# microsoft/MaskFlownet

Hardware: NVIDIA H100
Metric: image-pairs/sec (MaskFlownet-S forward, 1024x448) (higher is better)
Workload: dtype f32

## Files before the change

maskflownet_b200/csrc/conv3x3_wgmma.cu:

```cuda
#include <cstring>
#include <type_traits>

#include "mma_tiles.cuh"
#include "split_act.cuh"

namespace mfn {
namespace um {
constexpr int MT_WIDE = 128, MT_NARROW = 64;
inline int tile_width(int OW, int stride) {
  return tuning().conv_narrow && (OW <= MT_NARROW || (stride == 2 && tuning().conv_tma_in)) ? MT_NARROW : MT_WIDE;
}
constexpr int R = 2;
constexpr int NTHREADS = 384;
constexpr int NCONS = 8;
constexpr int NPROD = 3;
constexpr int MAX_AS = 4, MAX_WS = 24;
constexpr int MAX_RS = 4;
constexpr int BATCH = 6;
constexpr int BAR_BYTES = 1024;

__host__ __device__ inline int n_slots(int stride, int dil) { return stride == 2 ? 2 * R + 1 : (dil >= R ? 3 * R : R + 2 * dil); }
__host__ __device__ inline int row_pitch(int mt, int stride, int dil) { return stride == 2 ? 2 * mt + 1 : mt + 2 * dil; }
__host__ __device__ inline int slot_of(int r, int ky, int stride, int dil) {
  return stride == 2 ? 2 * r + ky : (dil >= R ? ky * R + r : r + ky * dil);
// ... 51 lines not shown
      : "+f"(d[0]), "+f"(d[1]), "+f"(d[2]), "+f"(d[3]), "+f"(d[4]), "+f"(d[5]), "+f"(d[6]), "+f"(d[7]), "+f"(d[8]), "+f"(d[9]), "+f"(d[10]), "+f"(d[11]), "+f"(d[12]), "+f"(d[13]), "+f"(d[14]), "+f"(d[15]), "+f"(d[16]), "+f"(d[17]), "+f"(d[18]), "+f"(d[19]), "+f"(d[20]), "+f"(d[21]), "+f"(d[22]), "+f"(d[23])
      : "l"(a), "l"(b), "r"(scale_d));
}
template <int S>
__device__ __forceinline__ void wgmma_n64(float (&d)[S], uint64_t a, uint64_t b, uint32_t scale_d) {
  static_assert(S >= 32, "accumulator too small");
  asm volatile(
      "{\n\t.reg .pred p;\n\tsetp.ne.b32 p, %34, 0;\n\t"
      "wgmma.mma_async.sync.aligned.m64n64k16.f32.bf16.bf16 {%0, %1, %2, %3, %4, %5, %6, %7, %8, %9, %10, %11, %12, %13, %14, %15, %16, %17, %18, %19, %20, %21, %22, %23, %24, %25, %26, %27, %28, %29, %30, %31}, %32, %33, p, 1, 1, 0, 0;\n\t}"
      : "+f"(d[0]), "+f"(d[1]), "+f"(d[2]), "+f"(d[3]), "+f"(d[4]), "+f"(d[5]), "+f"(d[6]), "+f"(d[7]), "+f"(d[8]), "+f"(d[9]), "+f"(d[10]), "+f"(d[11]), "+f"(d[12]), "+f"(d[13]), "+f"(d[14]), "+f"(d[15]), "+f"(d[16]), "+f"(d[17]), "+f"(d[18]), "+f"(d[19]), "+f"(d[20]), "+f"(d[21]), "+f"(d[22]), "+f"(d[23]), "+f"(d[24]), "+f"(d[25]), "+f"(d[26]), "+f"(d[27]), "+f"(d[28]), "+f"(d[29]), "+f"(d[30]), "+f"(d[31])
      : "l"(a), "l"(b), "r"(scale_d));
}
template <int S>
__device__ __forceinline__ void wgmma_n80(float (&d)[S], uint64_t a, uint64_t b, uint32_t scale_d) {
  static_assert(S >= 40, "accumulator too small");
  asm volatile(
      "{\n\t.reg .pred p;\n\tsetp.ne.b32 p, %42, 0;\n\t"
      "wgmma.mma_async.sync.aligned.m64n80k16.f32.bf16.bf16 {%0, %1, %2, %3, %4, %5, %6, %7, %8, %9, %10, %11, %12, %13, %14, %15, %16, %17, %18, %19, %20, %21, %22, %23, %24, %25, %26, %27, %28, %29, %30, %31, %32, %33, %34, %35, %36, %37, %38, %39}, %40, %41, p, 1, 1, 0, 0;\n\t}"
      : "+f"(d[0]), "+f"(d[1]), "+f"(d[2]), "+f"(d[3]), "+f"(d[4]), "+f"(d[5]), "+f"(d[6]), "+f"(d[7]), "+f"(d[8]), "+f"(d[9]), "+f"(d[10]), "+f"(d[11]), "+f"(d[12]), "+f"(d[13]), "+f"(d[14]), "+f"(d[15]), "+f"(d[16]), "+f"(d[17]), "+f"(d[18]), "+f"(d[19]), "+f"(d[20]), "+f"(d[21]), "+f"(d[22]), "+f"(d[23]), "+f"(d[24]), "+f"(d[25]), "+f"(d[26]), "+f"(d[27]), "+f"(d[28]), "+f"(d[29]), "+f"(d[30]), "+f"(d[31]), "+f"(d[32]), "+f"(d[33]), "+f"(d[34]), "+f"(d[35]), "+f"(d[36]), "+f"(d[37]), "+f"(d[38]), "+f"(d[39])
      : "l"(a), "l"(b), "r"(scale_d));
}
template <int S>
__device__ __forceinline__ void wgmma_n96(float (&d)[S], uint64_t a, uint64_t b, uint32_t scale_d) {
  static_assert(S >= 48, "accumulator too small");
  asm volatile(
      "{\n\t.reg .pred p;\n\tsetp.ne.b32 p, %50, 0;\n\t"
      "wgmma.mma_async.sync.aligned.m64n96k16.f32.bf16.bf16 {%0, %1, %2, %3, %4, %5, %6, %7, %8, %9, %10, %11, %12, %13, %14, %15, %16, %17, %18, %19, %20, %21, %22, %23, %24, %25, %26, %27, %28, %29, %30, %31, %32, %33, %34, %35, %36, %37, %38, %39, %40, %41, %42, %43, %44, %45, %46, %47}, %48, %49, p, 1, 1, 0, 0;\n\t}"
      : "+f"(d[0]), "+f"(d[1]), "+f"(d[2]), "+f"(d[3]), "+f"(d[4]), "+f"(d[5]), "+f"(d[6]), "+f"(d[7]), "+f"(d[8]), "+f"(d[9]), "+f"(d[10]), "+f"(d[11]), "+f"(d[12]), "+f"(d[13]), "+f"(d[14]), "+f"(d[15]), "+f"(d[16]), "+f"(d[17]), "+f"(d[18]), "+f"(d[19]), "+f"(d[20]), "+f"(d[21]), "+f"(d[22]), "+f"(d[23]), "+f"(d[24]), "+f"(d[25]), "+f"(d[26]), "+f"(d[27]), "+f"(d[28]), "+f"(d[29]), "+f"(d[30]), "+f"(d[31]), "+f"(d[32]), "+f"(d[33]), "+f"(d[34]), "+f"(d[35]), "+f"(d[36]), "+f"(d[37]), "+f"(d[38]), "+f"(d[39]), "+f"(d[40]), "+f"(d[41]), "+f"(d[42]), "+f"(d[43]), "+f"(d[44]), "+f"(d[45]), "+f"(d[46]), "+f"(d[47])
      : "l"(a), "l"(b), "r"(scale_d));
}
template <int S>
__device__ __forceinline__ void wgmma_n112(float (&d)[S], uint64_t a, uint64_t b, uint32_t scale_d) {
  static_assert(S >= 56, "accumulator too small");
  asm volatile(
      "{\n\t.reg .pred p;\n\tsetp.ne.b32 p, %58, 0;\n\t"
      "wgmma.mma_async.sync.aligned.m64n112k16.f32.bf16.bf16 {%0, %1, %2, %3, %4, %5, %6, %7, %8, %9, %10, %11, %12, %13, %14, %15, %16, %17, %18, %19, %20, %21, %22, %23, %24, %25, %26, %27, %28, %29, %30, %31, %32, %33, %34, %35, %36, %37, %38, %39, %40, %41, %42, %43, %44, %45, %46, %47, %48, %49, %50, %51, %52, %53, %54, %55}, %56, %57, p, 1, 1, 0, 0;\n\t}"
      : "+f"(d[0]), "+f"(d[1]), "+f"(d[2]), "+f"(d[3]), "+f"(d[4]), "+f"(d[5]), "+f"(d[6]), "+f"(d[7]), "+f"(d[8]), "+f"(d[9]), "+f"(d[10]), "+f"(d[11]), "+f"(d[12]), "+f"(d[13]), "+f"(d[14]), "+f"(d[15]), "+f"(d[16]), "+f"(d[17]), "+f"(d[18]), "+f"(d[19]), "+f"(d[20]), "+f"(d[21]), "+f"(d[22]), "+f"(d[23]), "+f"(d[24]), "+f"(d[25]), "+f"(d[26]), "+f"(d[27]), "+f"(d[28]), "+f"(d[29]), "+f"(d[30]), "+f"(d[31]), "+f"(d[32]), "+f"(d[33]), "+f"(d[34]), "+f"(d[35]), "+f"(d[36]), "+f"(d[37]), "+f"(d[38]), "+f"(d[39]), "+f"(d[40]), "+f"(d[41]), "+f"(d[42]), "+f"(d[43]), "+f"(d[44]), "+f"(d[45]), "+f"(d[46]), "+f"(d[47]), "+f"(d[48]), "+f"(d[49]), "+f"(d[50]), "+f"(d[51]), "+f"(d[52]), "+f"(d[53]), "+f"(d[54]), "+f"(d[55])
      : "l"(a), "l"(b), "r"(scale_d));
}
template <int S>
__device__ __forceinline__ void wgmma_n128(float (&d)[S], uint64_t a, uint64_t b, uint32_t scale_d) {
  static_assert(S >= 64, "accumulator too small");
  asm volatile(
      "{\n\t.reg .pred p;\n\tsetp.ne.b32 p, %66, 0;\n\t"
      "wgmma.mma_async.sync.aligned.m64n128k16.f32.bf16.bf16 {%0, %1, %2, %3, %4, %5, %6, %7, %8, %9, %10, %11, %12, %13, %14, %15, %16, %17, %18, %19, %20, %21, %22, %23, %24, %25, %26, %27, %28, %29, %30, %31, %32, %33, %34, %35, %36, %37, %38, %39, %40, %41, %42, %43, %44, %45, %46, %47, %48, %49, %50, %51, %52, %53, %54, %55, %56, %57, %58, %59, %60, %61, %62, %63}, %64, %65, p, 1, 1, 0, 0;\n\t}"
      : "+f"(d[0]), "+f"(d[1]), "+f"(d[2]), "+f"(d[3]), "+f"(d[4]), "+f"(d[5]), "+f"(d[6]), "+f"(d[7]), "+f"(d[8]), "+f"(d[9]), "+f"(d[10]), "+f"(d[11]), "+f"(d[12]), "+f"(d[13]), "+f"(d[14]), "+f"(d[15]), "+f"(d[16]), "+f"(d[17]), "+f"(d[18]), "+f"(d[19]), "+f"(d[20]), "+f"(d[21]), "+f"(d[22]), "+f"(d[23]), "+f"(d[24]), "+f"(d[25]), "+f"(d[26]), "+f"(d[27]), "+f"(d[28]), "+f"(d[29]), "+f"(d[30]), "+f"(d[31]), "+f"(d[32]), "+f"(d[33]), "+f"(d[34]), "+f"(d[35]), "+f"(d[36]), "+f"(d[37]), "+f"(d[38]), "+f"(d[39]), "+f"(d[40]), "+f"(d[41]), "+f"(d[42]), "+f"(d[43]), "+f"(d[44]), "+f"(d[45]), "+f"(d[46]), "+f"(d[47]), "+f"(d[48]), "+f"(d[49]), "+f"(d[50]), "+f"(d[51]), "+f"(d[52]), "+f"(d[53]), "+f"(d[54]), "+f"(d[55]), "+f"(d[56]), "+f"(d[57]), "+f"(d[58]), "+f"(d[59]), "+f"(d[60]), "+f"(d[61]), "+f"(d[62]), "+f"(d[63])
      : "l"(a), "l"(b), "r"(scale_d));
}
template <int N, int S>
__device__ __forceinline__ void wgmma_bf16(float (&d)[S], uint64_t a, uint64_t b, uint32_t scale_d) {
  if constexpr (N == 16) wgmma_n16(d, a, b, scale_d);
  else if constexpr (N == 32) wgmma_n32(d, a, b, scale_d);
  else if constexpr (N == 48) wgmma_n48(d, a, b, scale_d);
  else if constexpr (N == 64) wgmma_n64(d, a, b, scale_d);
  else if constexpr (N == 80) wgmma_n80(d, a, b, scale_d);
  else if constexpr (N == 96) wgmma_n96(d, a, b, scale_d);
  else if constexpr (N == 112) wgmma_n112(d, a, b, scale_d);
  else wgmma_n128(d, a, b, scale_d);
}

struct SplitK {
  int k, from, n_lo, y_lo, rh;
  long long part_stride;
  float* ws;
  uint32_t magic_tp, magic_tx;
  int as_wide;
  int ns;
  int stg;
};
__device__ __forceinline__ void decode_tile(int tile, int tilesX, int tilesY, const SplitK& sk, int& tx, int& ty, int& n) {
  if (sk.magic_tp) {
    n = (int)__umulhi((uint32_t)tile, sk.magic_tp);
    const int rem = tile - n * tilesX * tilesY;
    ty = sk.magic_tx ? (int)__umulhi((uint32_t)rem, sk.magic_tx) : rem;
    tx = rem - ty * tilesX;
  } else {
    tx = tile % tilesX;
    ty = (tile / tilesX) % tilesY;
    n = tile / (tilesX * tilesY);
  }
}
struct SplitDev {
  int in, in_g0, in_Cg;
  unsigned char* out;
  int out_Cg, out_c0;
};
struct Work {
  int tile, part, cb, ce, nh;
};
__device__ __forceinline__ Work decode_work(int w, const SplitK& sk, int nChunks) {
  Work r;
  r.nh = 0;
  if (sk.ns == 2) {
    r.nh = w & 1;
    w >>= 1;
  }
  if (sk.k <= 1 || w < sk.from) {
    r.tile = w; r.part = -1; r.cb = 0; r.ce = nChunks;
  } else {
    const int u = w - sk.from, t = u / sk.k;
    r.tile = sk.from + t;
    r.part = u - t * sk.k;
    r.cb = r.part * nChunks / sk.k;
    r.ce = (r.part + 1) * nChunks / sk.k;
  }
  return r;
}

struct SmemMap {
  int a_lo, a_stage, w_tile, w_stage, w_off, bar_off, stg_off, total, AS, WS, raw_off, raw_stage, RS;
};
constexpr int STG_CH = 32, SPITCH = MT_WIDE + 4;
constexpr int STG_BYTES = R * STG_CH * SPITCH * 4;
__host__ __device__ inline SmemMap smem_map(int E, int CoutP, int as_wide = 3, int stg = 0, int terms = 3, int raw = 0,
                                            int rs_max = 2) {
  SmemMap m;
  m.a_lo = 2 * E * 16;
  m.a_stage = terms == 1 ? m.a_lo : 2 * m.a_lo;
  m.w_tile = terms == 1 ? 32 * CoutP : 64 * CoutP;
  int budget = 227 * 1024 - BAR_BYTES - stg;
  m.w_stage = taps_per_stage(CoutP) * m.w_tile;
  m.RS = 0;
  if (raw) {
    const int raw_off = (2 * m.a_stage + 127) / 128 * 128;
    m.RS = rs_max;
    while (m.RS > 2 && budget - raw_off - m.RS * raw < 3 * m.w_stage) --m.RS;
    budget -= m.RS * raw + (raw_off - 2 * m.a_stage);
  }
  if (raw)
    m.AS = 2;
  else if (taps_per_stage(CoutP) > 1)
    m.AS = (4 * m.a_stage + 4 * m.w_stage <= budget) ? 4 : ((3 * m.a_stage + 3 * m.w_stage <= budget) ? 3 : 2);
  else
    m.AS = (as_wide >= 3 && 3 * m.a_stage + 8 * m.w_stage <= budget) ? 3 : 2;
  int ws = (budget - m.AS * m.a_stage) / m.w_stage;
  m.WS = ws > MAX_WS ? MAX_WS : ws;
  m.raw_off = raw ? (m.AS * m.a_stage + 127) / 128 * 128 : m.AS * m.a_stage;
  m.raw_stage = raw;
  m.w_off = m.raw_off + m.RS * raw;
  m.bar_off = m.w_off + m.WS * m.w_stage;
  m.stg_off = m.bar_off + BAR_BYTES;
  m.total = m.stg_off + stg;
  return m;
}
}

__global__ void conv3x3_pack_wgmma_kernel(const float* __restrict__ w, unsigned char* __restrict__ packed, int Cin, int Cout,
                                          int CoutP, int nChunks16) {
  const long long total = (long long)nChunks16 * 9 * CoutP * 8;
  for (long long i = (long long)blockIdx.x * blockDim.x + threadIdx.x; i < total; i += (long long)gridDim.x * blockDim.x) {
    const int j = (int)(i & 7);
    const int f = (int)((i >> 3) % CoutP);
    const int tap = (int)((i / (8LL * CoutP)) % 9);
    const int c = (int)(i / (8LL * CoutP * 9));
    const int ch = 16 * c + 2 * j;
    float a = 0.f, b = 0.f;
    if (f < Cout) {
      if (ch < Cin) a = w[((size_t)f * Cin + ch) * 9 + tap];
      if (ch + 1 < Cin) b = w[((size_t)f * Cin + ch + 1) * 9 + tap];
    }
    uint32_t hi, lo;
    split_pair(a, b, hi, lo);
    const int wt = 64 * CoutP;
    unsigned char* tile = packed + ((size_t)c * 9 + tap) * wt;
    if (um::fold_hi_lo(CoutP)) {
      const int off = (j >> 2) * (2 * CoutP * 16) + f * 16 + (j & 3) * 4;
// ... 202 lines not shown
        } else
#pragma unroll
        for (int pc = 0; pc < NCOL / SCH; ++pc) {
          if (t < SCH) bulk_wait_read();
          named_bar_sync(1 + r, 128);
#pragma unroll
          for (int jj = 0; jj < SCH / 8; ++jj) {
            const int j = pc * (SCH / 8) + jj;
#pragma unroll
            for (int e = 0; e < 2; ++e) {
              const int f = wk.nh * NCOL + 8 * j + 2 * (lane & 3) + e;
              const float b = (bias != nullptr && f < Cout) ? __ldg(bias + f) : 0.f;
              const float sl = f < lin_prefix ? 1.f : slope;
              float* const row = stg + (8 * jj + 2 * (lane & 3) + e) * SPITCH + 16 * wq + (lane >> 2);
#pragma unroll
              for (int mh = 0; mh < MB; ++mh)
#pragma unroll
                for (int h = 0; h < 2; ++h) {
                  const int i = 4 * j + 2 * h + e;
                  float v = acc[mh][i];
                  if constexpr (FOLD_ACC) v += acc[mh][i + NW / 4];
                  row[64 * mh + 8 * h] = leaky(v + b, sl);
                }
            }
          }
          asm volatile("fence.proxy.async.shared::cta;" ::: "memory");
          named_bar_sync(1 + r, 128);
          const int f = wk.nh * NCOL + pc * SCH + t;
          if (t < SCH && f < Cout) {
            bulk_s2g(out + (size_t)f * oplane0 + (size_t)y * OW + x0, smem_u32(stg + t * SPITCH), seg);
            bulk_commit();
          }
        }
      } else if (y < OH && !(dbg & 4)) {
#pragma unroll
        for (int mh = 0; mh < MB; ++mh) {
#pragma unroll
          for (int h = 0; h < 2; ++h) {
            const int xx = tx * MT + 64 * mh + 16 * wq + (lane >> 2) + 8 * h;
            if (xx >= OW) continue;
#pragma unroll
            for (int j = 0; j < NCOL / 8; ++j) {
#pragma unroll
              for (int e = 0; e < 2; ++e) {
                const int i = 4 * j + 2 * h + e;
                float v = acc[mh][i];
                if constexpr (FOLD_ACC) v += acc[mh][i + NW / 4];
                const int f = wk.nh * NCOL + 8 * j + 2 * (lane & 3) + e;
                if (f >= Cout) continue;
                if (xs.out != nullptr && !partial && f >= lin_prefix) {
                  if (e == 0) {
                    const float b0 = bias != nullptr ? __ldg(bias + f) : 0.f, b1 = bias != nullptr ? __ldg(bias + f + 1) : 0.f;
                    float v1 = acc[mh][i + 1];
                    if constexpr (FOLD_ACC) v1 += acc[mh][i + 1 + NW / 4];
                    sa::put_pair<P>(xs.out, xs.out_Cg, oplane0, n, xs.out_c0 + f - lin_prefix, (size_t)y * OW + xx,
                                 leaky(v + b0, slope), leaky(v1 + b1, slope));
                  }
                } else if (out_mode == 0) {
                  const float t = v + (bias != nullptr ? __ldg(bias + f) : 0.f);
                  out[(size_t)f * oplane0 + (size_t)y * OW + xx] = leaky(t, f < lin_prefix ? 1.f : slope);
                } else {
                  const int ph = f / F, ff = f - ph * F;
                  const float t = v + (bias != nullptr ? __ldg(bias + ff) : 0.f);
                  out[(size_t)ff * oplane2 + (size_t)(2 * y + (ph >> 1)) * (2 * OW) + 2 * xx + (ph & 1)] = leaky(t, slope);
                }
              }
            }
          }
        }
      }
    }
    bulk_wait_all();
  } else if (warp == 8) {
    if (lane == 0) {
      uint32_t ws = 0, wph = 0;
      bool wrapped = false;
      for (int work = blockIdx.x; work < numWork; work += gridDim.x) {
        const Work wk = decode_work(work, sk, nChunks);
        const int cb = wk.cb, ce = wk.ce;
        if constexpr (TERMS == 3) {
          const unsigned char* src = wpack + (size_t)cb * 9 * sm.w_tile;
          for (int it = 9 * cb; it < 9 * ce; it += TPS, src += sm.w_stage) {
            if (wrapped) mbar_wait(w_empty + 8 * ws, wph ^ 1);
            mbar_arrive_expect_tx(w_full + 8 * ws, (uint32_t)sm.w_stage);
            bulk_g2s(s_base + (uint32_t)sm.w_off + ws * (uint32_t)sm.w_stage, src, (uint32_t)sm.w_stage, w_full + 8 * ws);
            if (++ws == (uint32_t)WS) { ws = 0; wph ^= 1; wrapped = true; }
          }
        } else {
          const int gt = 64 * CoutP, run = 16 * CoutP;
          const unsigned char* src = wpack + (size_t)cb * 9 * gt;
          for (int it = 9 * cb; it < 9 * ce; it += TPS, src += TPS * gt) {
            if (wrapped) mbar_wait(w_empty + 8 * ws, wph ^ 1);
            mbar_arrive_expect_tx(w_full + 8 * ws, (uint32_t)sm.w_stage);
            const uint32_t dst = s_base + (uint32_t)sm.w_off + ws * (uint32_t)sm.w_stage;
#pragma unroll 1
            for (int t = 0; t < TPS; ++t) {
              if constexpr (FOLD) {
                bulk_g2s(dst + (uint32_t)(t * sm.w_tile), src + t * gt, (uint32_t)run, w_full + 8 * ws);
                bulk_g2s(dst + (uint32_t)(t * sm.w_tile + run), src + t * gt + 2 * run, (uint32_t)run, w_full + 8 * ws);
              } else {
                bulk_g2s(dst + (uint32_t)(t * sm.w_tile), src + t * gt, (uint32_t)sm.w_tile, w_full + 8 * ws);
              }
            }
            if (++ws == (uint32_t)WS) { ws = 0; wph ^= 1; wrapped = true; }
          }
        }
      }
    }
  } else {
    if (xs.in == 1) {
      if (warp == 9 && lane == 0) {
        uint32_t as = 0, aph = 0;
        bool wrapped = false;
        for (int work = blockIdx.x; work < numWork; work += gridDim.x) {
          const Work wk = decode_work(work, sk, nChunks);
          int tx, ty, n;
          decode_tile(wk.tile, tilesX, tilesY, sk, tx, ty, n);
          const int x0 = tx * MT - dil, y0 = ty * R;
          const int gb = n * P * xs.in_Cg + xs.in_g0;
          for (int c = wk.cb; c < wk.ce; ++c) {
            if (wrapped) mbar_wait(a_empty + 8 * as, aph ^ 1);
            const uint32_t bar = a_full + 8 * as, dst = s_base + as * (uint32_t)sm.a_stage;
            if (dbg & 16) {
              mbar_arrive(bar);
            } else {
              mbar_arrive_expect_tx(bar, (uint32_t)sm.a_stage);
              const int g = gb + 2 * c;
              if (dil < R) {
                tma_load_4d(dst, &tmx, 0, x0, y0 - dil, g, bar);
                if constexpr (P == 2) tma_load_4d(dst + (uint32_t)sm.a_lo, &tmx, 0, x0, y0 - dil, g + xs.in_Cg, bar);
              } else if constexpr (P == 1) {
#pragma unroll 1
                for (int k = 0; k < 6; ++k) {
                  const int ky = k >> 1, kc = k & 1;
                  tma_load_4d(dst + (uint32_t)((kc * E + ky * R * PW) * 16), &tmx, 0, x0, y0 + (ky - 1) * dil, g + kc, bar);
                }
              } else {
#pragma unroll 1
                for (int k = 0; k < 12; ++k) {
                  const int ky = k >> 2, kc = (k >> 1) & 1, pl = k & 1;
                  tma_load_4d(dst + (uint32_t)(pl * sm.a_lo + (kc * E + ky * R * PW) * 16), &tmx, 0, x0, y0 + (ky - 1) * dil,
                              g + kc + pl * xs.in_Cg, bar);
                }
              }
            }
            if (++as == (uint32_t)AS) { as = 0; aph ^= 1; wrapped = true; }
          }
        }
      }
      return;
    }
    if (dbg & 16) {
      uint32_t as = 0, aph = 0;
      bool wrapped = false;
      for (int work = blockIdx.x; work < numWork; work += gridDim.x) {
        const Work wk = decode_work(work, sk, nChunks);
        for (int c = wk.cb; c < wk.ce; ++c) {
          if (wrapped) mbar_wait(a_empty + 8 * as, aph ^ 1);
          __syncwarp();
          if (lane == 0) mbar_arrive(a_full + 8 * as);
          if (++as == (uint32_t)AS) { as = 0; aph ^= 1; wrapped = true; }
        }
      }
      return;
    }
    const int pw = warp - 9;
    const int G = (E + 31) / 32;
    const bool one_plane = Cin <= 8;
    const int nItems = one_plane ? G : 2 * G;
    const int nb = (nItems + NPROD * BATCH - 1) / (NPROD * BATCH);
    const uint32_t pw_magic = 0xFFFFFFFFu / (uint32_t)PW + 1u;
    if (one_plane) {
      for (int st = 0; st < AS; ++st)
        for (int e = pw * 32 + lane; e < E; e += NPROD * 32) {
          unsigned char* d = smem + st * sm.a_stage + (E + e) * 16;
          *reinterpret_cast<uint4*>(d) = make_uint4(0u, 0u, 0u, 0u);
          if constexpr (P == 2) *reinterpret_cast<uint4*>(d + sm.a_lo) = make_uint4(0u, 0u, 0u, 0u);
        }
    }
    if (xs.in == 2) {
      const bool s2 = stride == 2;
      const int RP = raw_pitch(MT, stride), CP = nslots * RP;
      const int RPC = s2 && !one_plane ? 2 : 1;
      const uint32_t raw_bytes = (uint32_t)sm.raw_stage, raw_base = s_base + (uint32_t)sm.raw_off;
      const bool issuer = warp == 9 && lane == 0;
      int i_work = blockIdx.x, i_c = 0, i_h = 0, i_ce = 0, i_x = 0, i_y = 0, i_n = 0;
      auto i_tile = [&]() {
        if (i_work >= numWork) return;
        const Work wk = decode_work(i_work, sk, nChunks);
        int tx, ty;
        decode_tile(wk.tile, tilesX, tilesY, sk, tx, ty, i_n);
        i_c = wk.cb;
        i_ce = wk.ce;
        i_x = s2 ? 2 * tx * MT - 4 : tx * MT - 4;
        i_y = s2 ? 2 * ty * R - 1 : ty * R - 1;
      };
      auto issue = [&](uint32_t slot) {
        if (i_work >= numWork) return;
        const uint32_t bar = r_full + 8 * slot;
        if (dbg & 2) {
          mbar_arrive(bar);
        } else {
          mbar_arrive_expect_tx(bar, raw_bytes);
          tma_load_4d(raw_base + slot * raw_bytes, &tmx, i_x, i_y, 16 * i_c + 8 * i_h, i_n, bar);
        }
        if (++i_h < RPC) return;
        i_h = 0;
        if (++i_c >= i_ce) {
          i_work += gridDim.x;
          i_tile();
        }
      };
      if (issuer) {
        i_tile();
        for (int s = 0; s < RS; ++s) issue((uint32_t)s);
      }
      uint32_t as = 0, aph = 0, rs = 0, rph = 0;
      bool wrapped = false;
      for (int work = blockIdx.x; work < numWork; work += gridDim.x) {
        const Work wk = decode_work(work, sk, nChunks);
        for (int c = wk.cb; c < wk.ce; ++c) {
          unsigned char* a_st = smem + as * sm.a_stage;
          for (int h = 0; h < RPC; ++h) {
            mbar_wait(r_full + 8 * rs, rph);
            if (h == 0 && wrapped) mbar_wait(a_empty + 8 * as, aph ^ 1);
            const float* raw = reinterpret_cast<const float*>(smem + sm.raw_off + rs * raw_bytes);
// ... 185 lines not shown
  return check_launch("conv3x3_pack_wgmma_kernel");
}

template <int TERMS>
__global__ void conv3x3_wgmma_reduce_kernel(um::SplitK sk, um::SplitDev xs, int RN, const float* __restrict__ bias,
                                            float* __restrict__ out, long long out_bs, int Cout, int OH, int OW, float slope,
                                            int out_mode_arg) {
  const int out_mode = out_mode_arg & 0xff, lin_prefix = out_mode_arg >> 8;
  const long long total = (long long)RN * Cout * sk.rh * OW;
  const int F = Cout >> 2;
  for (long long i = (long long)blockIdx.x * blockDim.x + threadIdx.x; i < total; i += (long long)gridDim.x * blockDim.x) {
    float s = 0.f;
    for (int p = 0; p < sk.k; ++p) s += sk.ws[(size_t)p * (size_t)sk.part_stride + (size_t)i];
    const int x = (int)(i % OW), y = sk.y_lo + (int)((i / OW) % sk.rh), f = (int)((i / ((long long)OW * sk.rh)) % Cout);
    const int n = sk.n_lo + (int)(i / ((long long)OW * sk.rh * Cout));
    if (out_mode == 0) {
      const float b = bias ? __ldg(bias + f) : 0.f;
      const float v = leaky(s + b, f < lin_prefix ? 1.f : slope);
      if (xs.out != nullptr && f >= lin_prefix)
        sa::put_one<TERMS == 1 ? 1 : 2>(xs.out, xs.out_Cg, (long long)OH * OW, n, xs.out_c0 + f - lin_prefix, (long long)y * OW + x, v);
      else
        out[(size_t)n * out_bs + ((size_t)f * OH + y) * OW + x] = v;
    } else {
      const int ph = f / F, ff = f - ph * F;
      const float b = bias ? __ldg(bias + ff) : 0.f;
      out[(size_t)n * out_bs + ((size_t)ff * (2 * OH) + (2 * y + (ph >> 1))) * (2 * OW) + 2 * x + (ph & 1)] = leaky(s + b, slope);
    }
  }
}

static um::SplitK plan_split(int N, int Cin, int H, int W, int Cout, int stride, int dil, int grid_cap) {
  using namespace um;
  (void)dil;
  const int ns = cout_pad(Cout) > 128 ? 2 : 1;
  SplitK sk = {1, 0, 0, 0, 0, 0, nullptr, 0u, 0u, 3, ns};
  const int OH = (H - 1) / stride + 1, OW = (W - 1) / stride + 1, nChunks = (Cin + 15) / 16;
  const int MT = tile_width(OW, stride);
  const int tilesX = (OW + MT - 1) / MT, tilesY = (OH + R - 1) / R;
  const long long tiles = (long long)N * tilesX * tilesY;
  sk.from = (int)tiles;
  const int mode = tuning().conv_splitk;
  if (!mode || tiles >= (1 << 29)) return sk;
  const int sms = grid_cap > 0 && grid_cap < kNumSMs ? grid_cap : kNumSMs;
  const int kcap = mode > 1 ? mode : 32;
  if (2 * tiles * ns <= sms) {
    int k = (int)(sms / (tiles * ns));
    if (k > nChunks / 3) k = nChunks / 3;
    if (k > 8) k = 8;
    if (k > kcap) k = kcap;
    if (k >= 2) {
      sk.k = k; sk.from = 0; sk.n_lo = 0; sk.y_lo = 0; sk.rh = OH;
    }
  } else if (ns == 1 && tiles > sms) {
    const long long rounds = tiles / sms;
    long long tail = tiles - rounds * sms;
    tail = (tail + tilesX - 1) / tilesX * tilesX;
    int k = tail > 0 ? (int)(sms / tail) : 0;
    if (k > nChunks / 2) k = nChunks / 2;
    if (k > kcap) k = kcap;
    if (tail > 0 && tail <= (long long)tilesX * tilesY && rounds <= 12 && k >= 2 && nChunks >= 16 && Cout > 64) {
      sk.k = k; sk.from = (int)(tiles - tail); sk.n_lo = N - 1;
      sk.y_lo = (int)((sk.from / tilesX) % tilesY) * R;
      sk.rh = OH - sk.y_lo;
    }
  }
  if (sk.k > 1) sk.part_stride = (long long)(N - sk.n_lo) * Cout * sk.rh * OW;
  return sk;
}

long long conv3x3_wgmma_workspace_bytes(int N, int Cin, int H, int W, int Cout, int stride, int dil) {
  const um::SplitK sk = plan_split(N, Cin, H, W, Cout, stride, dil, tuning().conv_grid_cap);
  return sk.k > 1 ? sk.k * sk.part_stride * 4 : 0;
}

int conv3x3_wgmma_launch(const float* x, long long x_bs, const unsigned char* wpack, const float* bias, float* out,
                         long long out_bs, int N, int Cin, int H, int W, int Cout, int stride, int dil, int out_mode,
                         float slope, cudaStream_t st, int ext, float* ws, long long ws_bytes, const SplitIO& sio) {
  using namespace um;
  const int terms = (out_mode & MFN_CONV_BF16) ? 1 : 3;
  out_mode &= ~MFN_CONV_BF16;
  const int grow = ext == 2 ? 8 : 2 * ext;
  const int OH = stride == 2 ? (H - 1) / 2 + 1 : H + grow, OW = stride == 2 ? (W - 1) / 2 + 1 : W + grow;
  const int MT = tile_width(OW, stride);
  SplitDev xs = {0, 0, 0, nullptr, 0, 0};
  CUtensorMap tmx;
  memset(&tmx, 0, sizeof tmx);
  if (sio.in != nullptr) {
    if (stride != 1 || ext != 0 || sio.in_c0 % 16 != 0 || (dil >= R && dil % 2 != 0) || !aligned(sio.in, 16)) return -1;
    EncodeTiledFn fn = encode_tiled_fn();
    if (fn == nullptr) return fail(MFN_ERR_UNSUPPORTED, "cuTensorMapEncodeTiled is not available from this driver");
    const int Cg = sa::groups(sio.in_C);
    const cuuint64_t dim[4] = {8, (cuuint64_t)W, (cuuint64_t)H, (cuuint64_t)N * (terms == 1 ? 1 : 2) * Cg};
    const cuuint64_t strides[3] = {16, (cuuint64_t)W * 16, (cuuint64_t)W * H * 16};
    const cuuint32_t box[4] = {8, (cuuint32_t)row_pitch(MT, 1, dil), (cuuint32_t)(dil < R ? n_slots(1, dil) : R), dil < R ? 2u : 1u};
    const cuuint32_t es[4] = {1, 1, 1, 1};
    const CUresult r = fn(&tmx, CU_TENSOR_MAP_DATA_TYPE_BFLOAT16, 4, const_cast<void*>(sio.in), dim, strides, box, es,
                          CU_TENSOR_MAP_INTERLEAVE_NONE, CU_TENSOR_MAP_SWIZZLE_NONE, CU_TENSOR_MAP_L2_PROMOTION_L2_256B,
                          CU_TENSOR_MAP_FLOAT_OOB_FILL_NONE);
    if (r != CUDA_SUCCESS) return fail(MFN_ERR_UNSUPPORTED, "cuTensorMapEncodeTiled failed (CUresult %d)", (int)r);
    xs.in = 1;
    xs.in_g0 = sio.in_c0 / 8;
    xs.in_Cg = Cg;
  }
  if (sio.out != nullptr) {
    const int lp = out_mode >> 8;
    if ((out_mode & 0xff) != 0 || ext != 0 || sio.out_c0 % 16 != 0 || (Cout - lp) % 16 != 0 || lp % 2 != 0 ||
        sio.out_c0 + Cout - lp > sio.out_C || !aligned(sio.out, 16))
      return -1;
    xs.out = static_cast<unsigned char*>(sio.out);
    xs.out_Cg = sa::groups(sio.out_C);
    xs.out_c0 = sio.out_c0;
  }
  if (Cout > 256 || (stride != 1 && !(stride == 2 && dil == 1))) return -1;
  if (ext != 0 && !((ext == 1 || ext == 2) && stride == 1 && dil == 1 && out_mode == 0)) return -1;
  if ((out_mode >> 8) != 0 && (out_mode & 0xff) != 0) return -1;
  const int CoutP = um::cout_pad(Cout), nChunks = (Cin + 15) / 16;
  const int E = n_slots(stride, dil) * row_pitch(MT, stride, dil);
  const int as_wide = 3;
  const bool staged = (out_mode & 0xff) == 0 && ext == 0 &&
                      (xs.out != nullptr ? (out_mode >> 8) == 0 : OW % 4 == 0 && out_bs % 4 == 0 && aligned(out, 16)) &&
                      smem_map(E, CoutP, as_wide, STG_BYTES, terms).WS >= 2;
  int raw = 0;
  const bool raw_geometry = stride == 1 ? dil == 1 && MT == MT_WIDE : MT == MT_NARROW && OW > MT_NARROW;
  if (sio.in == nullptr && tuning().conv_tma_in && raw_geometry && ext == 0 && W % 4 == 0 && x_bs % 4 == 0 &&
      aligned(x, 16)) {
    raw = raw_stage_bytes(n_slots(stride, 1), MT, stride);
    if (smem_map(E, CoutP, as_wide, staged ? STG_BYTES : 0, terms, raw, raw_ring_max(stride)).WS < 3) raw = 0;
  }
  if (raw) {
    EncodeTiledFn fn = encode_tiled_fn();
    if (fn == nullptr) return fail(MFN_ERR_UNSUPPORTED, "cuTensorMapEncodeTiled is not available from this driver");
    const cuuint64_t dim[4] = {(cuuint64_t)W, (cuuint64_t)H, (cuuint64_t)Cin, (cuuint64_t)N};
    const cuuint64_t strides[3] = {(cuuint64_t)W * 4, (cuuint64_t)W * H * 4, (cuuint64_t)x_bs * 4};
    const cuuint32_t box[4] = {(cuuint32_t)raw_pitch(MT, stride), (cuuint32_t)n_slots(stride, 1),
                               (cuuint32_t)raw_channels(stride), 1};
    const cuuint32_t es[4] = {1, 1, 1, 1};
    const CUresult r = fn(&tmx, CU_TENSOR_MAP_DATA_TYPE_FLOAT32, 4, const_cast<float*>(x), dim, strides, box, es,
                          CU_TENSOR_MAP_INTERLEAVE_NONE, CU_TENSOR_MAP_SWIZZLE_NONE, CU_TENSOR_MAP_L2_PROMOTION_L2_256B,
                          CU_TENSOR_MAP_FLOAT_OOB_FILL_NONE);
    if (r != CUDA_SUCCESS) return fail(MFN_ERR_UNSUPPORTED, "cuTensorMapEncodeTiled failed (CUresult %d)", (int)r);
    xs.in = 2;
  }
  const SmemMap sm = smem_map(E, CoutP, as_wide, staged ? STG_BYTES : 0, terms, raw, raw_ring_max(stride));
  if (sm.WS < 2 || E * 16 > 0x3FFF * 16) return -1;
  if ((long long)H * W >= (1LL << 27)) return -1;
  const int tilesX = (OW + MT - 1) / MT, tilesY = (OH + R - 1) / R;
  const int ns = CoutP > 128 ? 2 : 1;
  SplitK sk = {1, 0, 0, 0, 0, 0, nullptr, 0u, 0u, 3, ns};
  if (ws != nullptr && ext == 0) {
    sk = plan_split(N, Cin, H, W, Cout, stride, dil, tuning().conv_grid_cap);
    if (sk.k > 1 && ws_bytes < sk.k * sk.part_stride * 4) sk.k = 1;
    sk.ws = ws;
  }
  const long long tiles = (long long)N * tilesX * tilesY;
  if (tiles * ns >= (1LL << 30)) return -1;
  sk.as_wide = as_wide;
  sk.stg = staged ? STG_BYTES : 0;
  if (sk.k <= 1) sk.from = (int)tiles;
  {
    const unsigned long long tp = (unsigned long long)tilesX * tilesY;
    if ((unsigned long long)tiles * tp < (1ull << 32) && tp * tilesX < (1ull << 32)) {
      sk.magic_tp = (uint32_t)(((1ull << 32) + tp - 1) / tp);
      sk.magic_tx = tilesX == 1 ? 0u : (uint32_t)(((1ull << 32) + tilesX - 1) / tilesX);
    }
    if (tp == 1) sk.magic_tp = 0;
  }
  const long long numWork = (sk.from + (tiles - sk.from) * sk.k) * ns;
  const int cap = tuning().conv_grid_cap > 0 ? tuning().conv_grid_cap : kNumSMs;
  const unsigned grid = (unsigned)(numWork < cap ? numWork : cap);
  const char* name = terms == 3 ? "conv3x3_wgmma_kernel<CoutP=256>" : "conv3x3_wgmma_kernel<CoutP=256,bf16>";
  auto launch = [&](auto mt) -> cudaError_t {
    constexpr int M = decltype(mt)::value;
    static SmemOptIn opt[8], opt1[8];
    cudaError_t e = cudaSuccess;
    if (terms == 3) {
      e = ensure_dyn_smem(conv3x3_wgmma_kernel<32, true, 9, 3, M>, sm.total, opt[0]);
      if (e == cudaSuccess) e = ensure_dyn_smem(conv3x3_wgmma_kernel<64, true, 9, 3, M>, sm.total, opt[1]);
      if (e == cudaSuccess) e = ensure_dyn_smem(conv3x3_wgmma_kernel<96, true, 3, 3, M>, sm.total, opt[2]);
      if (e == cudaSuccess) e = ensure_dyn_smem(conv3x3_wgmma_kernel<128, true, 3, 3, M>, sm.total, opt[3]);
      if (e == cudaSuccess) e = ensure_dyn_smem(conv3x3_wgmma_kernel<80, false, 1, 3, M>, sm.total, opt[4]);
      if (e == cudaSuccess) e = ensure_dyn_smem(conv3x3_wgmma_kernel<96, false, 1, 3, M>, sm.total, opt[5]);
      if (e == cudaSuccess) e = ensure_dyn_smem(conv3x3_wgmma_kernel<112, false, 1, 3, M>, sm.total, opt[6]);
      if (e == cudaSuccess) e = ensure_dyn_smem(conv3x3_wgmma_kernel<128, false, 1, 3, M>, sm.total, opt[7]);
    } else {
      e = ensure_dyn_smem(conv3x3_wgmma_kernel<16, true, 9, 1, M>, sm.total, opt1[0]);
// ... 59 lines not shown
```

Baseline: 821.0.

## Replace TMA tensor-map input loads with per-lane bulk row copies and manual padding

For split-activation inputs, the producer warp no longer issues TMA tiled loads through a CUtensorMap. Instead each lane owns one input row and channel plane: it zero-fills the out-of-bounds edges in shared memory and issues a 1D bulk copy for the in-bounds span, with the expected byte count computed by a warp ballot. This removes the host-side tensor-map encoding and spreads copy issue across 32 lanes instead of one thread, at the cost of more, smaller bulk copies, explicit zero-fill stores and proxy fences. It also adds a debug flag (dbg&32) that skips the weight loads.

```diff
diff --git a/maskflownet_b200/csrc/conv3x3_wgmma.cu b/maskflownet_b200/csrc/conv3x3_wgmma.cu
--- a/maskflownet_b200/csrc/conv3x3_wgmma.cu
+++ b/maskflownet_b200/csrc/conv3x3_wgmma.cu
@@ -157,6 +157,7 @@
 }
 struct SplitDev {
   int in, in_g0, in_Cg;
+  const unsigned char* in_buf;
   unsigned char* out;
   int out_Cg, out_c0;
 };
@@ -525,8 +526,12 @@
           const unsigned char* src = wpack + (size_t)cb * 9 * sm.w_tile;
           for (int it = 9 * cb; it < 9 * ce; it += TPS, src += sm.w_stage) {
             if (wrapped) mbar_wait(w_empty + 8 * ws, wph ^ 1);
-            mbar_arrive_expect_tx(w_full + 8 * ws, (uint32_t)sm.w_stage);
-            bulk_g2s(s_base + (uint32_t)sm.w_off + ws * (uint32_t)sm.w_stage, src, (uint32_t)sm.w_stage, w_full + 8 * ws);
+            if (dbg & 32) {
+              mbar_arrive(w_full + 8 * ws);
+            } else {
+              mbar_arrive_expect_tx(w_full + 8 * ws, (uint32_t)sm.w_stage);
+              bulk_g2s(s_base + (uint32_t)sm.w_off + ws * (uint32_t)sm.w_stage, src, (uint32_t)sm.w_stage, w_full + 8 * ws);
+            }
             if (++ws == (uint32_t)WS) { ws = 0; wph ^= 1; wrapped = true; }
           }
         } else {
@@ -534,6 +539,11 @@
           const unsigned char* src = wpack + (size_t)cb * 9 * gt;
           for (int it = 9 * cb; it < 9 * ce; it += TPS, src += TPS * gt) {
             if (wrapped) mbar_wait(w_empty + 8 * ws, wph ^ 1);
+            if (dbg & 32) {
+              mbar_arrive(w_full + 8 * ws);
+              if (++ws == (uint32_t)WS) { ws = 0; wph ^= 1; wrapped = true; }
+              continue;
+            }
             mbar_arrive_expect_tx(w_full + 8 * ws, (uint32_t)sm.w_stage);
             const uint32_t dst = s_base + (uint32_t)sm.w_off + ws * (uint32_t)sm.w_stage;
 #pragma unroll 1
@@ -552,39 +562,44 @@
     }
   } else {
     if (xs.in == 1) {
-      if (warp == 9 && lane == 0) {
+      if (warp == 9) {
         uint32_t as = 0, aph = 0;
         bool wrapped = false;
+        const long long HW = (long long)H * W;
+        const int ncp = nslots * 2 * P;
+        const int pl = lane % P, kc = (lane / P) & 1, s = lane / (2 * P);
+        const bool mine = lane < ncp;
+        const int ky = s / R, rr = s - ky * R;
         for (int work = blockIdx.x; work < numWork; work += gridDim.x) {
           const Work wk = decode_work(work, sk, nChunks);
           int tx, ty, n;
           decode_tile(wk.tile, tilesX, tilesY, sk, tx, ty, n);
           const int x0 = tx * MT - dil, y0 = ty * R;
-          const int gb = n * P * xs.in_Cg + xs.in_g0;
+          const int xa = x0 > 0 ? x0 : 0, xb = x0 + PW < W ? x0 + PW : W;
+          const int e0 = xa - x0, e1 = xb - x0;
+          const int y = dil < R ? y0 - dil + s : y0 + (ky - 1) * dil + rr;
+          const bool row_in = mine && (unsigned)y < (unsigned)H;
+          const uint32_t bytes = (uint32_t)__popc(__ballot_sync(0xffffffffu, row_in)) * (uint32_t)(e1 - e0) * 16u;
           for (int c = wk.cb; c < wk.ce; ++c) {
             if (wrapped) mbar_wait(a_empty + 8 * as, aph ^ 1);
-            const uint32_t bar = a_full + 8 * as, dst = s_base + as * (uint32_t)sm.a_stage;
+            const uint32_t bar = a_full + 8 * as;
             if (dbg & 16) {
-              mbar_arrive(bar);
+              if (lane == 0) mbar_arrive(bar);
             } else {
-              mbar_arrive_expect_tx(bar, (uint32_t)sm.a_stage);
-              const int g = gb + 2 * c;
-              if (dil < R) {
-                tma_load_4d(dst, &tmx, 0, x0, y0 - dil, g, bar);
-                if constexpr (P == 2) tma_load_4d(dst + (uint32_t)sm.a_lo, &tmx, 0, x0, y0 - dil, g + xs.in_Cg, bar);
-              } else if constexpr (P == 1) {
-#pragma unroll 1
-                for (int k = 0; k < 6; ++k) {
-                  const int ky = k >> 1, kc = k & 1;
-                  tma_load_4d(dst + (uint32_t)((kc * E + ky * R * PW) * 16), &tmx, 0, x0, y0 + (ky - 1) * dil, g + kc, bar);
-                }
-              } else {
-#pragma unroll 1
-                for (int k = 0; k < 12; ++k) {
-                  const int ky = k >> 2, kc = (k >> 1) & 1, pl = k & 1;
-                  tma_load_4d(dst + (uint32_t)(pl * sm.a_lo + (kc * E + ky * R * PW) * 16), &tmx, 0, x0, y0 + (ky - 1) * dil,
-                              g + kc + pl * xs.in_Cg, bar);
-                }
+              unsigned char* const row = smem + as * sm.a_stage + pl * sm.a_lo + (kc * E + s * PW) * 16;
+              if (mine) {
+                const int z0 = row_in ? e0 : PW;
+                for (int e = 0; e < z0; ++e) *reinterpret_cast<uint4*>(row + e * 16) = make_uint4(0u, 0u, 0u, 0u);
+                if (row_in)
+                  for (int e = e1; e < PW; ++e) *reinterpret_cast<uint4*>(row + e * 16) = make_uint4(0u, 0u, 0u, 0u);
+              }
+              asm volatile("fence.proxy.async.shared::cta;" ::: "memory");
+              __syncwarp();
+              if (lane == 0) mbar_arrive_expect_tx(bar, bytes);
+              __syncwarp();
+              if (row_in) {
+                const long long src = sa::entry<P>(n, pl, xs.in_g0 + 2 * c + kc, (long long)y * W + xa, xs.in_Cg, HW);
+                bulk_g2s(smem_u32(row + e0 * 16), xs.in_buf + src, (uint32_t)(e1 - e0) * 16u, bar);
               }
             }
             if (++as == (uint32_t)AS) { as = 0; aph ^= 1; wrapped = true; }
@@ -936,25 +951,15 @@
   const int grow = ext == 2 ? 8 : 2 * ext;
   const int OH = stride == 2 ? (H - 1) / 2 + 1 : H + grow, OW = stride == 2 ? (W - 1) / 2 + 1 : W + grow;
   const int MT = tile_width(OW, stride);
-  SplitDev xs = {0, 0, 0, nullptr, 0, 0};
+  SplitDev xs = {0, 0, 0, nullptr, nullptr, 0, 0};
   CUtensorMap tmx;
   memset(&tmx, 0, sizeof tmx);
   if (sio.in != nullptr) {
     if (stride != 1 || ext != 0 || sio.in_c0 % 16 != 0 || (dil >= R && dil % 2 != 0) || !aligned(sio.in, 16)) return -1;
-    EncodeTiledFn fn = encode_tiled_fn();
-    if (fn == nullptr) return fail(MFN_ERR_UNSUPPORTED, "cuTensorMapEncodeTiled is not available from this driver");
-    const int Cg = sa::groups(sio.in_C);
-    const cuuint64_t dim[4] = {8, (cuuint64_t)W, (cuuint64_t)H, (cuuint64_t)N * (terms == 1 ? 1 : 2) * Cg};
-    const cuuint64_t strides[3] = {16, (cuuint64_t)W * 16, (cuuint64_t)W * H * 16};
-    const cuuint32_t box[4] = {8, (cuuint32_t)row_pitch(MT, 1, dil), (cuuint32_t)(dil < R ? n_slots(1, dil) : R), dil < R ? 2u : 1u};
-    const cuuint32_t es[4] = {1, 1, 1, 1};
-    const CUresult r = fn(&tmx, CU_TENSOR_MAP_DATA_TYPE_BFLOAT16, 4, const_cast<void*>(sio.in), dim, strides, box, es,
-                          CU_TENSOR_MAP_INTERLEAVE_NONE, CU_TENSOR_MAP_SWIZZLE_NONE, CU_TENSOR_MAP_L2_PROMOTION_L2_256B,
-                          CU_TENSOR_MAP_FLOAT_OOB_FILL_NONE);
-    if (r != CUDA_SUCCESS) return fail(MFN_ERR_UNSUPPORTED, "cuTensorMapEncodeTiled failed (CUresult %d)", (int)r);
     xs.in = 1;
+    xs.in_buf = static_cast<const unsigned char*>(sio.in);
     xs.in_g0 = sio.in_c0 / 8;
-    xs.in_Cg = Cg;
+    xs.in_Cg = sa::groups(sio.in_C);
   }
   if (sio.out != nullptr) {
     const int lp = out_mode >> 8;
```

Result: faster. 846.6, median of 6 (+3.1%).
